# blasif/cocons

Hardware: AMD Instinct MI355X
Metric: -2loglik evals/sec (dense cov_rns + Cholesky/solve/log-det, fp64) at n=10000 (higher is better)
Workload: dtype f64

## Files before the change

cocons_amd/csrc/chol.hip:

```cpp
#include <hip/hip_runtime.h>
#include <limits.h>
#include <stdlib.h>
#include <string.h>
#include <algorithm>
#include <atomic>
#include <vector>
#include "kernels.h"

namespace cocons {

typedef double d4 __attribute__((ext_vector_type(4)));

#define MFMA64(a, b, c) __builtin_amdgcn_mfma_f64_16x16x4f64((a), (b), (c), 0, 0, 0)
#define MFMA64_NEGA(a, b, c) __builtin_amdgcn_mfma_f64_16x16x4f64((a), (b), (c), 0, 0, 1)

__device__ __forceinline__ void blk_mma(d4 &acc, const d4 &P, const d4 &Q)
{
    acc = MFMA64(Q[0], P[0], acc);
    acc = MFMA64(Q[1], P[1], acc);
    acc = MFMA64(Q[2], P[2], acc);
    acc = MFMA64(Q[3], P[3], acc);
}

__device__ __forceinline__ d4 lds_blk(const double *blk, int lane)
{
    d4 v;
    int o = (lane >> 4) * 16 + (lane & 15);
    v[0] = blk[o];
    v[1] = blk[o + 64];
    v[2] = blk[o + 128];
    v[3] = blk[o + 192];
    return v;
}

__device__ __forceinline__ void lds_blk_store(double *blk, int lane, const d4 &v)
{
    int o = (lane >> 4) * 16 + (lane & 15);
    blk[o] = v[0];
    blk[o + 64] = v[1];
    blk[o + 128] = v[2];
    blk[o + 192] = v[3];
}

__device__ __forceinline__ d4 glb_blk(const double *A, size_t lda, int row0, int col0, int lane)
{
    const double *p = A + (size_t)(row0 + (lane & 15)) + (size_t)(col0 + (lane >> 4)) * lda;
    d4 v;
    v[0] = p[0];
    v[1] = p[4 * lda];
    v[2] = p[8 * lda];
    v[3] = p[12 * lda];
    return v;
}

__device__ __forceinline__ void glb_blk_store(double *A, size_t lda, int row0, int col0, int lane, const d4 &v)
{
    double *p = A + (size_t)(row0 + (lane & 15)) + (size_t)(col0 + (lane >> 4)) * lda;
    p[0] = v[0];
    p[4 * lda] = v[1];
    p[8 * lda] = v[2];
    p[12 * lda] = v[3];
}

__device__ __forceinline__ void store_wt(double *p, double v)
{
    __hip_atomic_store((unsigned long long *)p, (unsigned long long)__double_as_longlong(v), __ATOMIC_RELAXED,
                       __HIP_MEMORY_SCOPE_AGENT);
}

__device__ __forceinline__ double load_wt(const double *p)
{
    return __longlong_as_double((long long)__hip_atomic_load((const unsigned long long *)p, __ATOMIC_RELAXED,
                                                             __HIP_MEMORY_SCOPE_AGENT));
}

__device__ __forceinline__ d4 glb_blk_wt(const double *A, size_t lda, int row0, int col0, int lane)
{
    const double *p = A + (size_t)(row0 + (lane & 15)) + (size_t)(col0 + (lane >> 4)) * lda;
    d4 v;
    v[0] = load_wt(p);
    v[1] = load_wt(p + 4 * lda);
    v[2] = load_wt(p + 8 * lda);
    v[3] = load_wt(p + 12 * lda);
    return v;
}

__device__ __forceinline__ void glb_blk_store_wt(double *A, size_t lda, int row0, int col0, int lane, const d4 &v)
{
    double *p = A + (size_t)(row0 + (lane & 15)) + (size_t)(col0 + (lane >> 4)) * lda;
    store_wt(p, v[0]);
    store_wt(p + 4 * lda, v[1]);
    store_wt(p + 8 * lda, v[2]);
    store_wt(p + 12 * lda, v[3]);
}

__device__ __forceinline__ double rdlane(double v, int lane)
{
    int lo = __builtin_amdgcn_readlane(__double2loint(v), lane);
    int hi = __builtin_amdgcn_readlane(__double2hiint(v), lane);
    return __hiloint2double(hi, lo);
}

__device__ __forceinline__ void rsqrt_pivot(double a, double &l, double &r)
{
    const double y0 = __builtin_amdgcn_rsq(a);
    const double s0 = a * y0;
    const double t = fma(-s0, y0, 1.0);
    const double y = fma(y0 * t, fma(t, 0.375, 0.5), y0);
    double s = a * y;
    s = fma(fma(-s, s, a), 0.5 * y, s);
    l = s;
    r = y;
}

__device__ __forceinline__ double sel_lower4(int c, int k, double v00, double v10, double v11, double v20,
                                             double v21, double v22, double v30, double v31, double v32, double v33)
{
    double r0 = v00;
    double r1 = (k == 0) ? v10 : v11;
    double r2 = (k == 0) ? v20 : ((k == 1) ? v21 : v22);
    double r3 = (k == 0) ? v30 : ((k == 1) ? v31 : ((k == 2) ? v32 : v33));
    double r = (c == 0) ? r0 : ((c == 1) ? r1 : ((c == 2) ? r2 : r3));
    return (k <= c) ? r : 0.0;
}

template <int S>
__device__ __forceinline__ void potrf16_step(d4 &D, double (&Q)[4], int lane, int &fail)
{
    const int m = lane & 15, k = lane >> 4;
    const double ds = D[S];
    double a00 = rdlane(ds, 4 * S + 0), a10 = rdlane(ds, 4 * S + 1), a20 = rdlane(ds, 4 * S + 2),
           a30 = rdlane(ds, 4 * S + 3);
    double a11 = rdlane(ds, 4 * S + 1 + 16), a21 = rdlane(ds, 4 * S + 2 + 16), a31 = rdlane(ds, 4 * S + 3 + 16);
    double a22 = rdlane(ds, 4 * S + 2 + 32), a32 = rdlane(ds, 4 * S + 3 + 32);
    double a33 = rdlane(ds, 4 * S + 3 + 48);
    double l00, r0;
    rsqrt_pivot(a00, l00, r0);
    double l10 = a10 * r0, l20 = a20 * r0, l30 = a30 * r0;
    double t11 = fma(-l10, l10, a11);
    double l11, r1;
    rsqrt_pivot(t11, l11, r1);
    double l21 = fma(-l20, l10, a21) * r1, l31 = fma(-l30, l10, a31) * r1;
    double t22 = fma(-l21, l21, fma(-l20, l20, a22));
    double l22, r2;
    rsqrt_pivot(t22, l22, r2);
    double l32 = fma(-l31, l21, fma(-l30, l20, a32)) * r2;
    double t33 = fma(-l32, l32, fma(-l31, l31, fma(-l30, l30, a33)));
    double l33, r3;
    rsqrt_pivot(t33, l33, r3);
    if (__builtin_amdgcn_ballot_w64(!(t33 > 0.0)) != 0ull && fail == 0)
        fail = 4 * S + (!(a00 > 0.0) ? 1 : (!(t11 > 0.0) ? 2 : (!(t22 > 0.0) ? 3 : 4)));
    double m00 = r0, m11 = r1, m22 = r2, m33 = r3;
    double m10 = -(l10 * m00) * r1;
    double m21 = -(l21 * m11) * r2;
    double m32 = -(l32 * m22) * r3;
    double m20 = -fma(l21, m10, l20 * m00) * r2;
    double m31 = -fma(l32, m21, l31 * m11) * r3;
    double m30 = -fma(l32, m20, fma(l31, m10, l30 * m00)) * r3;
    const int c = m & 3;
    const bool ingrp = (m >> 2) == S;
    double q = sel_lower4(c, k, m00, m10, m11, m20, m21, m22, m30, m31, m32, m33);
    q = ingrp ? q : 0.0;
    Q[S] = q;
    d4 z = {0.0, 0.0, 0.0, 0.0};
    d4 X = MFMA64(q, ds, z);
    (void)l11; (void)l22; (void)l33; (void)l00;
    double xs = (m < 4 * S + k) ? 0.0 : X[S];
    if (S < 3) {
        d4 U = MFMA64(xs, -xs, D);
#pragma unroll
        for (int r = S + 1; r < 4; ++r) D[r] = U[r];
    }
    D[S] = xs;
}

__device__ __forceinline__ int potrf16_regs(d4 &D, double (&Q)[4], int lane)
{
    int fail = 0;
    potrf16_step<0>(D, Q, lane, fail);
    potrf16_step<1>(D, Q, lane, fail);
    potrf16_step<2>(D, Q, lane, fail);
    potrf16_step<3>(D, Q, lane, fail);
    return fail;
}

__device__ __forceinline__ void trsm16(d4 &B, const d4 &L, const double (&Q)[4])
{
    const d4 z = {0.0, 0.0, 0.0, 0.0};
#pragma unroll
    for (int s = 0; s < 4; ++s) {
        d4 T = MFMA64(Q[s], B[s], z);
        B[s] = T[s];
        if (s < 3) {
            d4 U = MFMA64(L[s], -B[s], B);
#pragma unroll
            for (int r = s + 1; r < 4; ++r) B[r] = U[r];
        }
    }
}

__constant__ int c_tri_ib[36] = {0, 1, 1, 2, 2, 2, 3, 3, 3, 3, 4, 4, 4, 4, 4, 5, 5, 5, 5, 5, 5,
                                 6, 6, 6, 6, 6, 6, 6, 7, 7, 7, 7, 7, 7, 7, 7};

#ifndef POTRF_S_WAVES
#define POTRF_S_WAVES 7
#endif
#define MBOX_OFF(j) (256 * (9 * (j) - (j) * ((j) - 1) / 2))
__device__ __forceinline__ void mbox_store(double *mb, int lane, const d4 &v)
{
    store_wt(mb + lane, v[0]);
    store_wt(mb + lane + 64, v[1]);
    store_wt(mb + lane + 128, v[2]);
    store_wt(mb + lane + 192, v[3]);
}
template <bool WT, bool FROM_LDS = false>
__device__ __forceinline__ void potrf_tile_body(double *A, size_t lda, int c0, double *q_out, int *info, double *smem,
                                                double *qall, double *winv = nullptr, double *xi = nullptr, double *mbox = nullptr,
                                                unsigned *late = nullptr)
{
    const bool INV = winv != nullptr;
    double *S = smem;
    double *QS = smem + 36 * 256;
#define SB(ib, kb) (S + ((ib) * ((ib) + 1) / 2 + (kb)) * 256)
    int tid_ = threadIdx.x;
    asm volatile("" : "+v"(tid_));
    const int tid = tid_, lane = tid & 63, wave = __builtin_amdgcn_readfirstlane(tid >> 6);

    d4 D0 = {0.0, 0.0, 0.0, 0.0};
    double Q0[4] = {0.0, 0.0, 0.0, 0.0};
    if (FROM_LDS) {
        if (wave == 0) {
            D0 = lds_blk(S, lane);
            int f = potrf16_regs(D0, Q0, lane);
            if (f && lane == 0) atomicMin(info, c0 + f);
        }
    } else {
    if (wave == 0) {
#pragma unroll
        for (int r = 0; r < 4; ++r) {
            const int i = lane & 15, c = 4 * r + (lane >> 4);
            const double *sp = i < c ? A + (size_t)(c0 + c) + (size_t)(c0 + i) * lda : A + (size_t)(c0 + i) + (size_t)(c0 + c) * lda;
            D0[r] = WT ? load_wt(sp) : *sp;
        }
    }
    {
        const int i = tid & 15, k = (tid >> 4) & 15;
        const int half = __builtin_amdgcn_readfirstlane(tid >> 8);
        const double *src = A + (size_t)(c0 + i) + (size_t)(c0 + k) * lda;
        const double *srcd = (i < k) ? A + (size_t)(c0 + k) + (size_t)(c0 + i) * lda : src;
        double v[18];
#pragma unroll
        for (int t = 0; t < 18; ++t) {
            const int bb = 2 * t + half;
            const int ib = c_tri_ib[bb], kb = bb - ib * (ib + 1) / 2;
            const double *sp = (ib == kb ? srcd : src) + (size_t)(16 * ib) + (size_t)(16 * kb) * lda;
            v[t] = WT ? load_wt(sp) : *sp;
        }
        if (wave == 0) {
            int f = potrf16_regs(D0, Q0, lane);
            if (f && lane == 0) atomicMin(info, c0 + f);
        }
#pragma unroll
        for (int t = 0; t < 18; ++t) {
            const int bb = 2 * t + half;
            const int ib = c_tri_ib[bb], kb = bb - ib * (ib + 1) / 2;
            SB(ib, kb)[k * 16 + i] = v[t];
        }
    }
    }
    __syncthreads();
    if (wave == 0) {
        lds_blk_store(S, lane, D0);
        if (WT) glb_blk_store_wt(A, lda, c0, c0, lane, D0); else glb_blk_store(A, lda, c0, c0, lane, D0);
        if (mbox) mbox_store(mbox, lane, D0);
#pragma unroll
        for (int s = 0; s < 4; ++s) {
            QS[s * 64 + lane] = Q0[s];
            if (WT) store_wt(q_out + s * 64 + lane, Q0[s]); else q_out[s * 64 + lane] = Q0[s];
            if (qall) qall[s * 64 + lane] = Q0[s];
            if (mbox) store_wt(mbox + 8 * 256 + s * 64 + lane, Q0[s]);
        }
    }
    __syncthreads();

    for (int jb = 0; jb < 7; ++jb) {
        double *dblk = SB(jb, jb);
        double *qs = QS;
        if (jb + 1 + wave < 8) {
            const int ib = jb + 1 + wave;
            d4 L = lds_blk(dblk, lane);
            double Q[4];
#pragma unroll
            for (int s = 0; s < 4; ++s) Q[s] = qs[s * 64 + lane];
            double *blk = SB(ib, jb);
            d4 B = lds_blk(blk, lane);
            trsm16(B, L, Q);
            lds_blk_store(blk, lane, B);
            if (WT) glb_blk_store_wt(A, lda, c0 + 16 * ib, c0 + 16 * jb, lane, B);
            else glb_blk_store(A, lda, c0 + 16 * ib, c0 + 16 * jb, lane, B);
            if (mbox) mbox_store(mbox + MBOX_OFF(jb) + (ib - jb) * 256, lane, B);
        }
        __syncthreads();
        if (wave == 0) {
            const int nb = jb + 1;
            d4 P = lds_blk(SB(nb, jb), lane);
            double *blk = SB(nb, nb);
            d4 acc = lds_blk(blk, lane);
            d4 NP = -P;
            blk_mma(acc, NP, P);
            double Q[4];
            int f = potrf16_regs(acc, Q, lane);
            if (f && lane == 0) atomicMin(info, c0 + 16 * nb + f);
            if (late && jb == 0) asm volatile("s_waitcnt vmcnt(0)" ::: "memory");
            lds_blk_store(blk, lane, acc);
            if (WT) glb_blk_store_wt(A, lda, c0 + 16 * nb, c0 + 16 * nb, lane, acc);
            else glb_blk_store(A, lda, c0 + 16 * nb, c0 + 16 * nb, lane, acc);
            if (mbox) mbox_store(mbox + MBOX_OFF(nb), lane, acc);
// ... 958 lines not shown
        if (((row / (2 * TILE) / own_group) % own_world) != own_rank) return;
    }
    if (wait_word) {
        if (tid == 0) ok = wait_ge<false>(wait_word, 1u, abort_word, abort_code(ABORT_PANEL, (unsigned)(c0 / TILE))) ? 1 : 0;
        asm volatile("s_waitcnt vmcnt(0)" ::: "memory");
        __syncthreads();
        if (!ok) return;
        fetch_factor_tile<true>(A, lda, c0, qin, SL, QS, tid);
    } else
        fetch_factor_tile<false>(A, lda, c0, qin, SL, QS, tid);
    const int bx = blockIdx.x;
    const int rs = (bx < nb1 ? r0 + 64 * bx : e0 + 64 * (bx - nb1)) + 16 * wave;
    d4 B[8];
#pragma unroll
    for (int j = 0; j < 8; ++j) B[j] = glb_blk(A, lda, rs, c0 + 16 * j, lane);
    __syncthreads();
#pragma unroll
    for (int j = 0; j < 8; ++j) {
        d4 L = lds_blk(SL + (j * (j + 1) / 2 + j) * 256, lane);
        double Q[4];
#pragma unroll
        for (int s = 0; s < 4; ++s) Q[s] = QS[j * 256 + s * 64 + lane];
        trsm16(B[j], L, Q);
        d4 NX = -B[j];
#pragma unroll
        for (int jj = j + 1; jj < 8; ++jj) {
            d4 Lb = lds_blk(SL + (jj * (jj + 1) / 2 + j) * 256, lane);
            blk_mma(B[jj], NX, Lb);
        }
    }
#pragma unroll
    for (int j = 0; j < 8; ++j) glb_blk_store(A, lda, rs, c0 + 16 * j, lane, B[j]);
}


struct UpdArgs {
    double *C; size_t ldc;
    const double *P; size_t ldp;
    int K;
    int ti0, tj0, lower_only;
    int H, W;
    unsigned *sig; int sig_tile;
    unsigned *wait_word, *abort_word;
    int ptiles, world, rank;
    const int *pmap;
    int skip_lo, skip_hi;
    unsigned *queue; unsigned ntiles;
    int Hb, ext0;
    int c_wt;
    int skew, kblk;
};

template <int TM, int KC, int ROLE, int NW = 4>
__global__ void __launch_bounds__(64 * NW, 8)
update_kernel(UpdArgs a)
{
    constexpr int LDT = TM + 16;
    constexpr int WY = NW / 2;
    constexpr int NB = TM / 32;
    constexpr int NBY = TM / WY / 16;
    constexpr int TPC = 64 * NW / KC;
    constexpr int RPT = TM / TPC;
    __shared__ double sI[2][KC * LDT];
    __shared__ double sJ[2][KC * LDT];
    unsigned *share = (unsigned *)&sI[0][TM];
    const int tid = threadIdx.x;
    const int wave_s = __builtin_amdgcn_readfirstlane(tid >> 6);
    if (a.wait_word) {
        if (tid == 0) *share = wait_ge(a.wait_word, 1u, a.abort_word, abort_code(ABORT_INPANEL, (unsigned)a.tj0)) ? 1u : 0u;
        asm volatile("s_waitcnt vmcnt(0)" ::: "memory");
        __syncthreads();
        const unsigned ok = *share;
        __syncthreads();
        if (!ok) return;
    }

    else if (a.abort_word) {
        if (tid == 0) *share = __hip_atomic_load(a.abort_word, __ATOMIC_RELAXED, __HIP_MEMORY_SCOPE_AGENT);
        __syncthreads();
        const unsigned ab = *share;
        __syncthreads();
        if (ab) return;
    }

    const int nch = a.K / KC;
    typedef double d2 __attribute__((ext_vector_type(2)));

    unsigned L = blockIdx.x;
    for (;;) {
        int lane;
        asm volatile("v_mbcnt_lo_u32_b32 %0, -1, 0\n\tv_mbcnt_hi_u32_b32 %0, -1, %0" : "=v"(lane));
        const int wave = wave_s, t2 = 64 * wave + lane;
        const int wi = wave & 1, wj = wave >> 1;
        const int kc = t2 / TPC, rg = (t2 % TPC) * RPT;
        const int ro = (lane >> 4) * LDT + (lane & 15);
        int ti, tj;
        if (a.lower_only) {
            int lo = 0, hi = a.W - 1;
            while (lo < hi) {
                const int mid = (lo + hi + 1) >> 1;
                if (mid * a.H - mid * (mid - 1) / 2 <= (int)L) lo = mid; else hi = mid - 1;
            }
            const int j = lo;
            const int til = j + ((int)L - (j * a.H - j * (j - 1) / 2));
            tj = a.tj0 + j;
            ti = til < a.Hb ? a.tj0 + til : a.ext0 + (til - a.Hb);
        } else {
            const int til = blockIdx.x;
            ti = til < a.Hb ? a.ti0 + til : a.ext0 + (til - a.Hb);
            tj = a.tj0 + blockIdx.y;
        }
        if (a.world > 1 && ((ti * TM / (2 * TILE) / a.ptiles) % a.world) != a.rank) return;
        if (ti >= a.skip_lo && ti < a.skip_hi && tj >= a.skip_lo && tj < a.skip_hi) {
            if (!a.queue) return;
            if (t2 == 0) *share = gridDim.x + __hip_atomic_fetch_add(a.queue, 1u, __ATOMIC_RELAXED, __HIP_MEMORY_SCOPE_AGENT);
            __syncthreads();
            L = (unsigned)__builtin_amdgcn_readfirstlane((int)*share);
            __syncthreads();
            if (L >= a.ntiles) break;
            continue;
        }
        const int sig_Ti = (ti * TM) / TILE - a.sig_tile, sig_Tj = (tj * TM) / TILE - a.sig_tile;
        const bool sig_wg = a.sig != nullptr && sig_Ti >= 0 && sig_Ti <= 1 && sig_Tj >= 0 && sig_Tj <= sig_Ti;
        const bool wt_wg = sig_wg || a.c_wt;
        if (sig_wg) __builtin_amdgcn_s_setprio(3); else __builtin_amdgcn_s_setprio(0);

        int rowI_P = ti * TM, rowJ_P = tj * TM, rowI_C = ti * TM;
        if (a.pmap) { rowI_P = a.pmap[ti]; rowJ_P = a.pmap[tj]; }
        if (a.skew) {
            const bool ext = ti >= a.ext0;
            const int under = a.skew * TILE + (ti - a.ext0) * TM;
            rowI_P = ext ? under : ti * TM - TILE * a.kblk;
            rowJ_P = tj * TM - TILE * a.kblk;
            rowI_C = ext ? under : ti * TM - TILE * ((tj * TM) / TILE);
        }
        const double *gI = a.P + (size_t)(rowI_P + rg) + (size_t)kc * a.ldp;
        const double *gJ = a.P + (size_t)(rowJ_P + rg) + (size_t)kc * a.ldp;
        d2 stI[RPT / 2], stJ[RPT / 2];

        double *Cb = a.C + (size_t)(rowI_C + (TM / 2) * wi) + (size_t)(tj * TM + (TM / WY) * wj) * a.ldc;
        const unsigned ldcb = 8u * (unsigned)a.ldc;
        const unsigned cvo = 8u * (unsigned)(lane & 15) + (unsigned)(lane >> 4) * ldcb;
        d4 acc[NB][NBY];
#pragma unroll
        for (int x = 0; x < NB; ++x)
#pragma unroll
            for (int y = 0; y < NBY; ++y) acc[x][y] = (d4){0.0, 0.0, 0.0, 0.0};

#pragma unroll
        for (int v = 0; v < RPT / 2; ++v) {
            stI[v] = *(const d2 *)(gI + 2 * v);
            stJ[v] = *(const d2 *)(gJ + 2 * v);
        }
#pragma unroll
        for (int v = 0; v < RPT / 2; ++v) {
            *(d2 *)(&sI[0][kc * LDT + rg + 2 * v]) = stI[v];
            *(d2 *)(&sJ[0][kc * LDT + rg + 2 * v]) = stJ[v];
        }
        __syncthreads();

        for (int ch = 0; ch < nch; ++ch) {
            const int cur = ch & 1;
            if (ch + 1 < nch) {
                const double *pI = gI + (size_t)(ch + 1) * KC * a.ldp;
                const double *pJ = gJ + (size_t)(ch + 1) * KC * a.ldp;
#pragma unroll
                for (int v = 0; v < RPT / 2; ++v) {
                    stI[v] = *(const d2 *)(pI + 2 * v);
                    stJ[v] = *(const d2 *)(pJ + 2 * v);
                }
            }
            const double *bI = &sI[cur][ro + (TM / 2) * wi];
            const double *bJ = &sJ[cur][ro + (TM / WY) * wj];
#pragma unroll
            for (int s = 0; s < KC / 4; ++s) {
                double pi_[NB], pj_[NBY];
#pragma unroll
                for (int x = 0; x < NB; ++x) pi_[x] = bI[s * 4 * LDT + 16 * x];
#pragma unroll
                for (int y = 0; y < NBY; ++y) pj_[y] = bJ[s * 4 * LDT + 16 * y];
#pragma unroll
                for (int x = 0; x < NB; ++x)
#pragma unroll
                    for (int y = 0; y < NBY; ++y) acc[x][y] = MFMA64(pj_[y], pi_[x], acc[x][y]);
            }
            if (ch + 1 < nch) {
#pragma unroll
                for (int v = 0; v < RPT / 2; ++v) {
                    *(d2 *)(&sI[cur ^ 1][kc * LDT + rg + 2 * v]) = stI[v];
                    *(d2 *)(&sJ[cur ^ 1][kc * LDT + rg + 2 * v]) = stJ[v];
                }
            }
            __syncthreads();
        }
        unsigned Lnext = 0;
        if (a.queue && t2 == 0)
            Lnext = gridDim.x + __hip_atomic_fetch_add(a.queue, 1u, __ATOMIC_RELAXED, __HIP_MEMORY_SCOPE_AGENT);
        unsigned cve = cvo;
        asm volatile("" : "+v"(cve));
#pragma unroll
        for (int x = 0; x < NB; ++x)
#pragma unroll
            for (int y = 0; y < NBY; ++y) {
                d4 cv;
#pragma unroll
                for (int r = 0; r < 4; ++r) {
                    const double *cp = (const double *)((const char *)(Cb + 16 * x) + (cve + (unsigned)(16 * y + 4 * r) * ldcb));
                    cv[r] = a.c_wt ? load_wt(cp) : *cp;
                }
                cv -= acc[x][y];
                if (wt_wg) {
#pragma unroll
                    for (int r = 0; r < 4; ++r)
                        store_wt((double *)((char *)(Cb + 16 * x) + (cve + (unsigned)(16 * y + 4 * r) * ldcb)), cv[r]);
                } else {
#pragma unroll
                    for (int r = 0; r < 4; ++r)
                        *(double *)((char *)(Cb + 16 * x) + (cve + (unsigned)(16 * y + 4 * r) * ldcb)) = cv[r];
                }
            }
        if (wt_wg) {
            asm volatile("s_waitcnt vmcnt(0)" ::: "memory");
            __syncthreads();
            if (t2 == 0 && sig_wg) signal_add(a.sig + a.sig_tile + sig_Ti);
        }
        if (!a.queue) break;
        if (t2 == 0) *share = Lnext;
        __syncthreads();
        L = (unsigned)__builtin_amdgcn_readfirstlane((int)*share);
        if (L >= a.ntiles) break;
    }
}

struct DagStep {
    unsigned base;
    unsigned near;
    unsigned tpos, nT;
    int H, W;
    int tj0;
    int k0, K;
    int nstrip, two;
    int need;
    int nd_next;
    int split;
    unsigned p2, p3;
};

struct DagArgs {
    double *A; size_t lda;
    double *P;
    const double *Wt;
    const DagStep *steps; int nsteps;
    unsigned ntasks;
    unsigned *queue;
    unsigned *tdone;
    unsigned *pdone; int pstride;
    unsigned *pall;
    double *partbuf;
    unsigned *dcount;
    unsigned *sig;
    unsigned *out, *xr;
    unsigned *abort_word;
    const unsigned *alive;
    unsigned xcc_quota;
    unsigned *hw;
    unsigned long long *trace;
    const unsigned *ftab;
    unsigned xcd_g;
    unsigned *xcnt;
};

constexpr unsigned DAG_XCD_LAG = 64u;
__device__ __forceinline__ unsigned dag_position(unsigned c, unsigned cls, unsigned g)
{
    return ((c >> g) << (g + 3u)) | (cls << g) | (c & ((1u << g) - 1u));
}

__device__ __forceinline__ bool dag_wait(const DagArgs &a, unsigned *word, unsigned need, unsigned code, unsigned L)
{
    const unsigned long long t0 = __builtin_amdgcn_s_memrealtime();
    for (unsigned it = 0;; ++it) {
        const unsigned v = poll_word(word, it);
        if (v >= need) break;
        if (__hip_atomic_load(a.abort_word, __ATOMIC_RELAXED, __HIP_MEMORY_SCOPE_AGENT) != 0u) return false;
        if (it > (unsigned)(ENGINE_TIMEOUT_TICKS / 100ull) ||
            ((it & 1023u) == 1023u && __builtin_amdgcn_s_memrealtime() - t0 > WALL_BACKSTOP_TICKS)) {
            if (__hip_atomic_exchange(a.abort_word, code, __ATOMIC_RELAXED, __HIP_MEMORY_SCOPE_AGENT) == 0u) {
                unsigned *d = a.queue + 8;
                d[0] = L; d[1] = code; d[2] = (unsigned)(word - a.queue); d[3] = need; d[4] = v;
                d[5] = (unsigned)(__builtin_amdgcn_s_memrealtime() - t0);
                d[6] = it;
            }
            return false;
        }
        __builtin_amdgcn_s_sleep(16);
    }
    __builtin_amdgcn_fence(__ATOMIC_ACQUIRE, "wavefront");
    return true;
}

__global__ void __launch_bounds__(256, 8)
dag_kernel(DagArgs a)
{
    constexpr int TM = 64, KC = 8, LDT = TM + 16, TPC = 256 / KC, RPT = TM / TPC;
    static_assert(RPT == 2, "one 16-byte load per thread, side and chunk");
    typedef double d2 __attribute__((ext_vector_type(2)));
    __shared__ double sI[2][KC * LDT];
    __shared__ double sJ[2][KC * LDT];
    unsigned *share = (unsigned *)&sI[0][TM];
    const int tid = threadIdx.x;
    const int wave_s = __builtin_amdgcn_readfirstlane(tid >> 6);
    const DagStep *__restrict__ steps = a.steps;
    const unsigned ldab = 8u * (unsigned)a.lda;
    int known = 0;
    const unsigned myx = (hw_where() >> 28) & 7u;
    const bool loyal = ((blockIdx.x >> 3) & 1u) == 0u;
    if (tid == 0) {
        bool take = true;
        if (a.xcc_quota) {
            const unsigned c = __hip_atomic_load(a.alive + 16 + myx, __ATOMIC_RELAXED, __HIP_MEMORY_SCOPE_AGENT);
            if (c) {
                const unsigned less = 7u * (c - 1u);
                const unsigned quota = a.xcc_quota > less + 8u ? a.xcc_quota - less : 8u;
                take = __hip_atomic_fetch_add(a.queue + 16 + myx, 1u, __ATOMIC_RELAXED, __HIP_MEMORY_SCOPE_AGENT) < quota;
            }
        }
        unsigned first = 0xffffffffu;
        if (take) {
            if (a.xcd_g) first = dag_position(__hip_atomic_fetch_add(a.xcnt + 32u * myx, 1u, __ATOMIC_RELAXED, __HIP_MEMORY_SCOPE_AGENT), myx, a.xcd_g);
            else first = __hip_atomic_fetch_add(a.queue, 1u, __ATOMIC_RELAXED, __HIP_MEMORY_SCOPE_AGENT);
        }
        share[1] = first;
        share[2] = 0u;
    }
    __syncthreads();
    unsigned L = (unsigned)__builtin_amdgcn_readfirstlane((int)share[1]);
    __syncthreads();
    if (L >= a.ntasks) return;
    for (;;) {
        int lo = 0, hi = a.nsteps - 1;
        while (lo < hi) {
            const int mid = (lo + hi + 1) >> 1;
            if (steps[mid].base <= L) lo = mid; else hi = mid - 1;
        }
        const int s = lo;
        const DagStep st = steps[s];
        const unsigned q = L - st.base;
        if (a.trace && tid == 0) {
            a.trace[4 * (size_t)L] = __builtin_amdgcn_s_memrealtime();
            if (a.hw) a.hw[2 * (size_t)L] = hw_where();
        }
        const int t = st.tj0 >> 1;
        const unsigned per_u = 2u * (unsigned)st.nstrip, nA = per_u + (unsigned)st.nd_next, perBC = st.two ? per_u : 0u;
        int tkind = -1;
        unsigned tu = 0, qt_u = q;
        if (q >= st.tpos) {
            if (q < st.tpos + nA) { tu = q - st.tpos; tkind = tu < per_u ? 0 : 3; }
            else if (q < st.p2) qt_u = q - nA;
            else if (q < st.p2 + perBC) { tu = q - st.p2; tkind = 1; }
            else if (q < st.p3) qt_u = q - nA - perBC;
            else if (q < st.p3 + perBC) { tu = q - st.p3; tkind = 2; }
            else qt_u = q - nA - 2u * perBC;
        }
        const bool isT = tkind >= 0;
        const double *gIb, *gJb;
        unsigned ldib, ldjb, ldob = ldab;
        int K, i_wt = 0, store_only = 0, strip_task = 0;
        double *Cb;
        const double *pa = nullptr;
        unsigned *w0 = nullptr, *w1 = nullptr, *w2 = nullptr, *we = nullptr, *we2 = nullptr, *dn;
        unsigned n0 = 0, n1 = 0, n2 = 0, ne = 0, dval = 0;
        int sigT = -1;
        int prio = 0;
        if (!isT) {
            const int qt = (int)qt_u;
            int ti, tj;
            if (a.ftab && qt >= (int)st.near) {
                const unsigned e = a.ftab[a.ftab[s] + (unsigned)(qt - (int)st.near)];
                tj = st.tj0 + (int)(e & 0xffffu); ti = st.tj0 + (int)(e >> 16);
            } else {
                int jl = 0, jh = st.W - 1;
                while (jl < jh) {
                    const int mid = (jl + jh + 1) >> 1;
                    if (mid * st.H - mid * (mid - 1) / 2 <= qt) jl = mid; else jh = mid - 1;
                }
                tj = st.tj0 + jl; ti = tj + (qt - (jl * st.H - jl * (jl - 1) / 2));
            }
            const double *Ps = s == 0 ? a.A : a.P;
            gIb = Ps + (size_t)ti * TM + (size_t)st.k0 * a.lda;
            gJb = Ps + (size_t)tj * TM + (size_t)st.k0 * a.lda;
            ldib = ldab; ldjb = ldab; K = st.K;
            Cb = a.A + (size_t)ti * TM + (size_t)tj * TM * a.lda;
            if (s > known) {
                w0 = a.pall + s; n0 = (unsigned)st.H;
                w1 = a.pdone + (size_t)s * a.pstride + (ti - st.tj0); n1 = (unsigned)st.need;
                w2 = a.pdone + (size_t)s * a.pstride + (tj - st.tj0); n2 = (unsigned)st.need;
            }
            we = a.tdone + (ti * (ti + 1) / 2 + tj); ne = (unsigned)s;
            dn = we; dval = (unsigned)s + 1u;
            const int Ti = (ti >> 1) - t, Tj = (tj >> 1) - t;
            if (Ti >= 0 && Ti <= st.two && Tj >= 0 && Tj <= Ti) {
                sigT = t + Ti; prio = 3;
                if (st.split) {
                    const int ta = ti - st.tj0, tb = tj - st.tj0, dd = ta * (ta + 1) / 2 + tb;
                    gIb += (size_t)TILE * a.lda; gJb += (size_t)TILE * a.lda; K = TILE;
                    pa = a.partbuf + ((size_t)(s & 1) * 16 + dd) * (TM * TM);
                    we2 = a.dcount + (size_t)s * 16 + dd;
                }
            }
        } else {
            const int per = 2 * st.nstrip;
            const size_t c_t = (size_t)t * TILE, c_t1 = c_t + TILE;
            prio = 2;
            const int stage = tkind;
            int strip = 0, h = 0, row64 = 0;
            if (stage != 3) {
                strip = (int)(tu >> 1); h = (int)(tu & 1u);
                row64 = st.tj0 + (st.two ? 4 : 2) + strip;
                strip_task = 1;
            }
            dn = a.pdone + (size_t)(s + 1) * a.pstride + strip;
            if (stage == 3) {
                const int dd = (int)tu - per;
                const int ta = c_tri_ib[dd], tb = dd - ta * (ta + 1) / 2;
                const int tj0n = st.tj0 + 4;
                const size_t k0n = (size_t)(s + 1) * 2 * TILE;
                gIb = a.P + (size_t)(tj0n + ta) * TM + k0n * a.lda; ldib = ldab;
                gJb = a.P + (size_t)(tj0n + tb) * TM + k0n * a.lda; ldjb = ldab;
                K = TILE;
                Cb = a.partbuf + ((size_t)((s + 1) & 1) * 16 + dd) * (TM * TM); store_only = 1; ldob = 8u * TM;
                w0 = a.pdone + (size_t)(s + 1) * a.pstride + ta; n0 = 2u;
                w1 = a.pdone + (size_t)(s + 1) * a.pstride + tb; n1 = 2u;
                dn = a.dcount + (size_t)(s + 1) * 16 + dd;
            } else if (stage == 0) {
                gIb = a.A + (size_t)row64 * TM + c_t * a.lda; ldib = ldab; i_wt = 1;
                gJb = a.Wt + (size_t)t * TILE * TILE + TM * h; ldjb = 8u * TILE;
                K = TM * (h + 1);
                Cb = a.P + (size_t)row64 * TM + (c_t + TM * h) * a.lda; store_only = 1;
                w0 = a.out + t; n0 = 1u;
                w1 = a.tdone + (row64 * (row64 + 1) / 2 + 2 * t); n1 = (unsigned)s + 1u;
                w2 = w1 + 1; n2 = n1;
            } else if (stage == 1) {
                gIb = a.P + (size_t)row64 * TM + c_t * a.lda; ldib = ldab;
                gJb = a.P + (c_t1 + TM * h) + c_t * a.lda; ldjb = ldab;
                K = TILE;
                Cb = a.A + (size_t)row64 * TM + (c_t1 + TM * h) * a.lda;
                w0 = dn; n0 = 2u;
                w1 = a.xr + t; n1 = 1u;
                we = a.tdone + (row64 * (row64 + 1) / 2 + 2 * (t + 1) + h); ne = (unsigned)s + 1u;
            } else {
                gIb = a.A + (size_t)row64 * TM + c_t1 * a.lda; ldib = ldab; i_wt = 1;
                gJb = a.Wt + (size_t)(t + 1) * TILE * TILE + TM * h; ldjb = 8u * TILE;
                K = TM * (h + 1);
                Cb = a.P + (size_t)row64 * TM + (c_t1 + TM * h) * a.lda; store_only = 1;
                w0 = dn; n0 = 4u;
                w1 = a.out + t + 1; n1 = 1u;
            }
        }
        if (prio == 3) __builtin_amdgcn_s_setprio(3);
        else if (prio == 2) __builtin_amdgcn_s_setprio(2);
        else __builtin_amdgcn_s_setprio(0);

        if (w0) {
            if (tid == 0) {
                unsigned ok;
                if (!isT) {
                    if (__hip_atomic_load(w0, __ATOMIC_RELAXED, __HIP_MEMORY_SCOPE_AGENT) >= n0) ok = 2u;
                    else ok = (dag_wait(a, w1, n1, abort_code(0xb00u, (unsigned)s), L) &&
                               dag_wait(a, w2, n2, abort_code(0xc00u, (unsigned)s), L)) ? 1u : 0u;
                } else {
                    bool o = dag_wait(a, w0, n0, abort_code(0xa00u, (unsigned)s), L);
                    if (o && w1) o = dag_wait(a, w1, n1, abort_code(0xb00u, (unsigned)s), L);
                    if (o && w2) o = dag_wait(a, w2, n2, abort_code(0xc00u, (unsigned)s), L);
                    ok = o ? 1u : 0u;
                }
                *share = ok;
            }
            asm volatile("s_waitcnt vmcnt(0)" ::: "memory");
            __syncthreads();
            const unsigned ok = (unsigned)__builtin_amdgcn_readfirstlane((int)*share);
            __syncthreads();
            if (!ok) return;
            if (ok == 2u) known = s;
        }

        if (a.trace && tid == 0) a.trace[4 * (size_t)L + 1] = __builtin_amdgcn_s_memrealtime();
        int lane;
        asm volatile("v_mbcnt_lo_u32_b32 %0, -1, 0\n\tv_mbcnt_hi_u32_b32 %0, -1, %0" : "=v"(lane));
        const int wave = wave_s, t2 = 64 * wave + lane;
        const int wi = wave & 1, wj = wave >> 1;
        const int kc = t2 / TPC, rg = (t2 % TPC) * RPT;
        const int ro = (lane >> 4) * LDT + (lane & 15);
        const char *pI = (const char *)gIb + (8u * (unsigned)rg + (unsigned)kc * ldib);
        const char *pJ = (const char *)gJb + (8u * (unsigned)rg + (unsigned)kc * ldjb);
        const unsigned cIb = (unsigned)KC * ldib, cJb = (unsigned)KC * ldjb;
        const int nch = K / KC;
        d2 stI, stJ;
        d4 acc[2][2];
#pragma unroll
        for (int x = 0; x < 2; ++x)
#pragma unroll
            for (int y = 0; y < 2; ++y) acc[x][y] = (d4){0.0, 0.0, 0.0, 0.0};
        if (i_wt) { stI[0] = load_wt((const double *)pI); stI[1] = load_wt((const double *)pI + 1); }
        else stI = *(const d2 *)pI;
        stJ = *(const d2 *)pJ;
        *(d2 *)(&sI[0][kc * LDT + rg]) = stI;
        *(d2 *)(&sJ[0][kc * LDT + rg]) = stJ;
        __syncthreads();
        for (int ch = 0; ch < nch; ++ch) {
            const int cur = ch & 1;
            if (ch + 1 < nch) {
                const char *qI = pI + (unsigned)(ch + 1) * cIb;
                const char *qJ = pJ + (unsigned)(ch + 1) * cJb;
                if (i_wt) { stI[0] = load_wt((const double *)qI); stI[1] = load_wt((const double *)qI + 1); }
                else stI = *(const d2 *)qI;
                stJ = *(const d2 *)qJ;
            }
            const double *bI = &sI[cur][ro + (TM / 2) * wi];
            const double *bJ = &sJ[cur][ro + (TM / 2) * wj];
#pragma unroll
            for (int k4 = 0; k4 < KC / 4; ++k4) {
                const double p0 = bI[k4 * 4 * LDT], p1 = bI[k4 * 4 * LDT + 16];
                const double q0 = bJ[k4 * 4 * LDT], q1 = bJ[k4 * 4 * LDT + 16];
                acc[0][0] = MFMA64(q0, p0, acc[0][0]);
                acc[0][1] = MFMA64(q1, p0, acc[0][1]);
                acc[1][0] = MFMA64(q0, p1, acc[1][0]);
                acc[1][1] = MFMA64(q1, p1, acc[1][1]);
            }
            if (ch + 1 < nch) {
                *(d2 *)(&sI[cur ^ 1][kc * LDT + rg]) = stI;
                *(d2 *)(&sJ[cur ^ 1][kc * LDT + rg]) = stJ;
            }
            __syncthreads();
        }
        if (t2 == 0) {
            unsigned Ln, c = 0u, cy = 0u, cls = 0u, y = 0u;
            unsigned help = 0u;
            if (a.xcd_g) {
                help = loyal ? 0u : share[2];
                cls = help ? help - 1u : myx;
                y = help ? myx : ((myx + 1u + L % 7u) & 7u);
                c = __hip_atomic_fetch_add(a.xcnt + 32u * cls, 1u, __ATOMIC_RELAXED, __HIP_MEMORY_SCOPE_AGENT);
                cy = __hip_atomic_load(a.xcnt + 32u * y, __ATOMIC_RELAXED, __HIP_MEMORY_SCOPE_AGENT);
                Ln = 0u;
            } else
                Ln = __hip_atomic_fetch_add(a.queue, 1u, __ATOMIC_RELAXED, __HIP_MEMORY_SCOPE_AGENT);
            unsigned ok = 1u;
            if (we) ok = dag_wait(a, we, ne, abort_code(0xd00u, (unsigned)s), L) ? 1u : 0u;
            if (ok && we2) ok = wait_ge<false>(we2, 1u, a.abort_word, abort_code(0xe00u, (unsigned)s)) ? 1u : 0u;
            if (a.xcd_g) {
                Ln = dag_position(c, cls, a.xcd_g);
                if (!help) share[2] = (!loyal && c > cy + DAG_XCD_LAG && dag_position(cy, y, a.xcd_g) < a.ntasks) ? y + 1u : 0u;
                else {
                    share[2] = (c + DAG_XCD_LAG / 2u < cy && dag_position(c + 1u, cls, a.xcd_g) < a.ntasks) ? help : 0u;
                    if (Ln >= a.ntasks) {
                        cls = myx;
                        c = __hip_atomic_fetch_add(a.xcnt + 32u * cls, 1u, __ATOMIC_RELAXED, __HIP_MEMORY_SCOPE_AGENT);
                        Ln = dag_position(c, cls, a.xcd_g);
                    }
                }
                if (Ln >= a.ntasks && cls == myx) {
                    for (unsigned d = 1; d < 8u && Ln >= a.ntasks; ++d) {
                        const unsigned z = (myx + d) & 7u;
                        if (dag_position(__hip_atomic_load(a.xcnt + 32u * z, __ATOMIC_RELAXED, __HIP_MEMORY_SCOPE_AGENT), z, a.xcd_g) < a.ntasks)
                            Ln = dag_position(__hip_atomic_fetch_add(a.xcnt + 32u * z, 1u, __ATOMIC_RELAXED, __HIP_MEMORY_SCOPE_AGENT), z, a.xcd_g);
                    }
                }
            }
            share[0] = ok; share[1] = Ln;
            if (a.trace) a.trace[4 * (size_t)L + 2] = __builtin_amdgcn_s_memrealtime();
        }
        asm volatile("s_waitcnt vmcnt(0)" ::: "memory");
        __syncthreads();
        const unsigned okE = share[0];
        const unsigned Lnext = share[1];
        if (!okE) return;
        double *Cw = (double *)((char *)(Cb + (TM / 2) * wi) + (size_t)((TM / 2) * wj) * ldob);
        unsigned cve = 8u * (unsigned)(lane & 15) + (unsigned)(lane >> 4) * ldob;
        asm volatile("" : "+v"(cve));
#pragma unroll
        for (int x = 0; x < 2; ++x)
#pragma unroll
            for (int y = 0; y < 2; ++y) {
                d4 cv;
                if (store_only) cv = acc[x][y];
                else {
#pragma unroll
                    for (int r = 0; r < 4; ++r)
                        cv[r] = load_wt((const double *)((const char *)(Cw + 16 * x) + (cve + (unsigned)(16 * y + 4 * r) * ldob)));
                    if (pa) {
                        const double *Pw = pa + (TM / 2) * wi + (TM / 2) * wj * TM;
                        int ln;
                        asm volatile("v_mbcnt_lo_u32_b32 %0, -1, 0\n\tv_mbcnt_hi_u32_b32 %0, -1, %0" : "=v"(ln));
                        const unsigned cvp = 8u * (unsigned)(ln & 15) + (unsigned)(ln >> 4) * (8u * TM);
                        d4 pv;
#pragma unroll
                        for (int r = 0; r < 4; ++r)
                            pv[r] = load_wt((const double *)((const char *)(Pw + 16 * x) + (cvp + (unsigned)(16 * y + 4 * r) * (8u * TM))));
                        cv -= pv + acc[x][y];
                    } else cv -= acc[x][y];
                }
#pragma unroll
                for (int r = 0; r < 4; ++r)
                    store_wt((double *)((char *)(Cw + 16 * x) + (cve + (unsigned)(16 * y + 4 * r) * ldob)), cv[r]);
            }
        asm volatile("s_waitcnt vmcnt(0)" ::: "memory");
        __syncthreads();
        if (t2 == 0) {
            if (sigT >= 0) signal_add(a.sig + sigT);
            if (dval) __hip_atomic_fetch_max(dn, dval, __ATOMIC_RELAXED, __HIP_MEMORY_SCOPE_AGENT);
            else if (__hip_atomic_fetch_add(dn, 1u, __ATOMIC_RELAXED, __HIP_MEMORY_SCOPE_AGENT) + 1u == (st.two ? 6u : 2u) && strip_task)
                __hip_atomic_fetch_add(a.pall + s + 1, 1u, __ATOMIC_RELAXED, __HIP_MEMORY_SCOPE_AGENT);
            if (a.trace) {
                a.trace[4 * (size_t)L + 3] = __builtin_amdgcn_s_memrealtime();
                if (a.hw) a.hw[2 * (size_t)L + 1] = hw_where();
            }
        }
        L = (unsigned)__builtin_amdgcn_readfirstlane((int)Lnext);
        if (L >= a.ntasks) break;
    }
}

__device__ __forceinline__ double block_sum(double v, double *red)
{
#pragma unroll
    for (int o = 32; o > 0; o >>= 1) v += __shfl_down(v, o, 64);
    int lane = threadIdx.x & 63, wave = threadIdx.x >> 6;
    if (lane == 0) red[wave] = v;
    __syncthreads();
    double t = 0.0;
    if (threadIdx.x == 0)
        for (int w = 0; w < (int)(blockDim.x >> 6); ++w) t += red[w];
    __syncthreads();
    return t;
}

__global__ void __launch_bounds__(1024)
finalize_kernel(const double *A, size_t lda, int c0, int c1, int n, int row0, int nr, double *out, int skew, int npad,
                const double *A2, int a2_cols)
{
    __shared__ double red[16];
    const int b = blockIdx.x;
    const int hi = c1 < n ? c1 : n;
    double s = 0.0;
    constexpr int U = 4;
    const int step = (int)blockDim.x;
    if (b == nr * nr) {
        for (int c = c0 + (int)threadIdx.x; c < hi; c += U * step) {
            double v[U];
#pragma unroll
            for (int q = 0; q < U; ++q) v[q] = (c + q * step < hi) ? A[band_index(c + q * step, c + q * step, lda, skew, npad)] : 1.0;
#pragma unroll
            for (int q = 0; q < U; ++q) s += log(v[q]);
        }
    } else {
        const int ra = row0 + b / nr, rb = row0 + b % nr;
        for (int c = c0 + (int)threadIdx.x; c < hi; c += U * step) {
            double va[U], vb[U];
#pragma unroll
            for (int q = 0; q < U; ++q) {
                const bool in = c + q * step < hi;
                const int cc = c + q * step;
                int below0 = 2 * TILE * (cc / (2 * TILE) + 1);
                if (npad > 0 && below0 > npad) below0 = npad;
                const bool in2 = A2 && cc >= 2 * TILE && cc < a2_cols;
                const double *Sa = (in2 && ra >= below0) ? A2 : A;
                const double *Sb = (in2 && rb >= below0) ? A2 : A;
                va[q] = in ? Sa[band_index(ra, cc, lda, skew, npad)] : 0.0;
                vb[q] = in ? Sb[band_index(rb, cc, lda, skew, npad)] : 0.0;
            }
#pragma unroll
            for (int q = 0; q < U; ++q) s += va[q] * vb[q];
        }
    }
    s = block_sum(s, red);
    if (threadIdx.x == 0) out[b == nr * nr ? 0 : 1 + b] = s;
}

__global__ void __launch_bounds__(256)
row_reduce_kernel(const double *A, size_t lda, int n, int rowy, int row0, int m,
                  double *scratch, int cchunk, int skew, int npad, const double *A2, int a2_cols)
{
    const int i = blockIdx.x * blockDim.x + threadIdx.x;
    const int cb = blockIdx.y * cchunk;
    const int ce = (cb + cchunk < n) ? cb + cchunk : n;
    if (i >= m) return;
    if (A2 && cb >= 2 * TILE && cb < a2_cols) A = A2;
    double s = 0.0, q = 0.0;
    for (int c = cb; c < ce; ++c) {
        double v = A[band_index(row0 + i, c, lda, skew, npad)];
        double y = A[band_index(rowy, c, lda, skew, npad)];
        s = fma(v, y, s);
        q = fma(v, v, q);
    }
    scratch[((size_t)blockIdx.y * 2 + 0) * m + i] = s;
    scratch[((size_t)blockIdx.y * 2 + 1) * m + i] = q;
}

__global__ void __launch_bounds__(256)
row_reduce_final_kernel(const double *scratch, int m, int nchunks, double *stoch, double *quad)
{
    const int i = blockIdx.x * blockDim.x + threadIdx.x;
    if (i >= m) return;
    double s = 0.0, q = 0.0;
    for (int c = 0; c < nchunks; ++c) {
        s += scratch[((size_t)c * 2 + 0) * m + i];
        q += scratch[((size_t)c * 2 + 1) * m + i];
    }
    stoch[i] = s;
    quad[i] = q;
}

__global__ void __launch_bounds__(256)
trmm_lower_kernel(const double *A, size_t lda, int n, const double *E, int lde, int nsim,
                  const double *trend, double *Y, int ldy)
{
    __shared__ double red[4][8][64];
    const int lane = threadIdx.x & 63, wave = threadIdx.x >> 6;
    const int rb = gridDim.x - 1 - blockIdx.x;
    const int i = rb * 64 + lane;
    const int kend = (rb + 1) * 64 < n ? (rb + 1) * 64 : n;
    for (int s0 = 0; s0 < nsim; s0 += 8) {
        double acc[8] = {0, 0, 0, 0, 0, 0, 0, 0};
        for (int k = wave; k < kend; k += 4) {
            double l = (i < n && k <= i) ? A[(size_t)i + (size_t)k * lda] : 0.0;
#pragma unroll
            for (int s = 0; s < 8; ++s)
                if (s0 + s < nsim) acc[s] = fma(l, E[(size_t)k + (size_t)(s0 + s) * lde], acc[s]);
        }
#pragma unroll
        for (int s = 0; s < 8; ++s) red[wave][s][lane] = acc[s];
        __syncthreads();
        if (wave == 0 && i < n) {
#pragma unroll
            for (int s = 0; s < 8; ++s)
                if (s0 + s < nsim)
                    Y[(size_t)i + (size_t)(s0 + s) * ldy] =
                        ((red[0][s][lane] + red[1][s][lane]) + (red[2][s][lane] + red[3][s][lane])) + trend[i];
        }
        __syncthreads();
    }
}

void launch_trmm_lower(const double *A, size_t lda, int n, const double *E, int lde, int nsim,
                       const double *trend, double *Y, int ldy, hipStream_t s)
{
    if (n <= 0 || nsim <= 0) return;
    hipLaunchKernelGGL(trmm_lower_kernel, dim3((n + 63) / 64), dim3(256), 0, s, A, lda, n, E, lde, nsim, trend, Y, ldy);
}

constexpr int BT_COLS = 64;
constexpr size_t BT_LDS_BYTES = (size_t)TILE * BT_COLS * sizeof(double);

__device__ __forceinline__ int bt_lds_index(int k, int j)
{
    return (((k >> 4) * (BT_COLS / 16) + (j >> 4)) << 8) + ((k & 15) << 4) + ((j ^ k) & 15);
}

__global__ void __launch_bounds__(256)
band_trmm_kernel(const double *A, size_t lda, int skew, int npad, const int *hi, int n, const double *E, int lde,
                 int nsim, const double *trend, double *Y, int ldy)
{
    extern __shared__ double Es[];
    const int I = blockIdx.x, s0 = blockIdx.y * BT_COLS;
    const int lane = threadIdx.x & 63, wave = threadIdx.x >> 6;
    int c0 = 0;
    if (hi) {
        int lo = 0, up = I;
        while (lo < up) {
            const int mid = (lo + up) >> 1;
            if (hi[mid] > I) up = mid; else lo = mid + 1;
        }
        c0 = lo;
    }
    d4 acc[2][4];
#pragma unroll
    for (int rb = 0; rb < 2; ++rb)
#pragma unroll
        for (int jb = 0; jb < 4; ++jb) acc[rb][jb] = d4{0.0, 0.0, 0.0, 0.0};
    const int row0 = I * TILE + 32 * wave;
    for (int c = c0; c <= I; ++c) {
        __syncthreads();
        for (int e = threadIdx.x; e < TILE * BT_COLS; e += 256) {
            const int k = e & (TILE - 1), j = e >> 7;
            const int gk = c * TILE + k, gj = s0 + j;
            Es[bt_lds_index(k, j)] = (gk < n && gj < nsim) ? E[(size_t)gk + (size_t)gj * lde] : 0.0;
        }
        __syncthreads();
        const double *Ac = skew ? A - (ptrdiff_t)TILE * c : A;
        const bool diag = c == I;
#pragma unroll
        for (int kb = 0; kb < TILE / 16; ++kb) {
            if (diag && kb > 2 * wave + 1) break;
            d4 P[2];
#pragma unroll
            for (int rb = 0; rb < 2; ++rb) {
                const int lb = 2 * wave + rb;
                if (diag && kb > lb) { P[rb] = d4{0.0, 0.0, 0.0, 0.0}; continue; }
                P[rb] = glb_blk(Ac, lda, row0 + 16 * rb, c * TILE + 16 * kb, lane);
                if (diag && kb == lb) {
#pragma unroll
                    for (int r = 0; r < 4; ++r)
                        if (4 * r + (lane >> 4) > (lane & 15)) P[rb][r] = 0.0;
                }
            }
#pragma unroll
            for (int jb = 0; jb < 4; ++jb) {
                const double *blk = Es + ((kb * (BT_COLS / 16) + jb) << 8);
                d4 Q;
#pragma unroll
                for (int r = 0; r < 4; ++r) {
                    const int k = (lane >> 4) + 4 * r, j = lane & 15;
                    Q[r] = blk[(k << 4) + ((j ^ k) & 15)];
                }
                blk_mma(acc[0][jb], P[0], Q);
                blk_mma(acc[1][jb], P[1], Q);
            }
        }
    }
#pragma unroll
    for (int rb = 0; rb < 2; ++rb) {
        const int i = row0 + 16 * rb + (lane & 15);
        if (i >= n) continue;
        const double t = trend[i];
#pragma unroll
        for (int jb = 0; jb < 4; ++jb)
#pragma unroll
            for (int r = 0; r < 4; ++r) {
                const int j = s0 + 16 * jb + 4 * r + (lane >> 4);
                if (j < nsim) Y[(size_t)i + (size_t)j * ldy] = acc[rb][jb][r] + t;
            }
    }
}

static void set_dynamic_lds_once(const void *kernel, size_t bytes, std::atomic<unsigned long long> &done_mask);
void launch_band_trmm(const double *A, size_t lda, int skew, int npad, const int *d_hi, int nt, int n, const double *E,
                      int lde, int nsim, const double *trend, double *Y, int ldy, hipStream_t s)
// ... 602 lines not shown
```

Baseline: 119.2.

## Stream DAG GEMM tiles via global_load_lds into a 4-deep LDS ring

Replaces the register-staged double-buffered load/store of the I and J panels in the DAG tile kernel with direct global-to-LDS loads (global_load_lds) into a four-slot ring with KC=4. Loads run three chunks ahead, tracked by vmcnt waits. Waves 0-1 fetch I and waves 2-3 fetch J, with an XOR swizzle on the LDS layout. This removes the VGPR round-trip and the LDS store instructions, and makes global latency hiding deeper. In exchange there are more barriers per K element, since each chunk now holds 4 instead of 8. Correctness depends on hand-managed waitcnt ordering, and the loop assumes nch is a multiple of RING.

New measurement: 124.2, median of 6. +4.2%, better.

```diff
diff --git a/cocons_amd/csrc/chol.hip b/cocons_amd/csrc/chol.hip
--- a/cocons_amd/csrc/chol.hip
+++ b/cocons_amd/csrc/chol.hip
@@ -13,6 +13,7 @@
 
 #define MFMA64(a, b, c) __builtin_amdgcn_mfma_f64_16x16x4f64((a), (b), (c), 0, 0, 0)
 #define MFMA64_NEGA(a, b, c) __builtin_amdgcn_mfma_f64_16x16x4f64((a), (b), (c), 0, 0, 1)
+#define LDS_T __attribute__((address_space(3)))
 
 __device__ __forceinline__ void blk_mma(d4 &acc, const d4 &P, const d4 &Q)
 {
@@ -1577,12 +1578,9 @@
 __global__ void __launch_bounds__(256, 8)
 dag_kernel(DagArgs a)
 {
-    constexpr int TM = 64, KC = 8, LDT = TM + 16, TPC = 256 / KC, RPT = TM / TPC;
-    static_assert(RPT == 2, "one 16-byte load per thread, side and chunk");
-    typedef double d2 __attribute__((ext_vector_type(2)));
-    __shared__ double sI[2][KC * LDT];
-    __shared__ double sJ[2][KC * LDT];
-    unsigned *share = (unsigned *)&sI[0][TM];
+    constexpr int TM = 64, KC = 4, RING = 4, STG = 2 * KC * TM;
+    __shared__ double smem[RING * STG + 2];
+    unsigned *share = (unsigned *)&smem[RING * STG];
     const int tid = threadIdx.x;
     const int wave_s = __builtin_amdgcn_readfirstlane(tid >> 6);
     const DagStep *__restrict__ steps = a.steps;
@@ -1764,50 +1762,52 @@
         asm volatile("v_mbcnt_lo_u32_b32 %0, -1, 0\n\tv_mbcnt_hi_u32_b32 %0, -1, %0" : "=v"(lane));
         const int wave = wave_s, t2 = 64 * wave + lane;
         const int wi = wave & 1, wj = wave >> 1;
-        const int kc = t2 / TPC, rg = (t2 % TPC) * RPT;
-        const int ro = (lane >> 4) * LDT + (lane & 15);
-        const char *pI = (const char *)gIb + (8u * (unsigned)rg + (unsigned)kc * ldib);
-        const char *pJ = (const char *)gJb + (8u * (unsigned)rg + (unsigned)kc * ldjb);
-        const unsigned cIb = (unsigned)KC * ldib, cJb = (unsigned)KC * ldjb;
+        const bool opJ = wave >= 2;
+        const char *gsrc = opJ ? (const char *)gJb : (const char *)gIb;
+        const unsigned ldg = opJ ? ldjb : ldib, cstep = (unsigned)KC * ldg;
+        const bool wt = i_wt && !opJ;
+        const int sc = (lane >> 5) & 1;
+        const char *src = gsrc + ((unsigned)(2 * (wave & 1) + sc) * ldg + 8u * (unsigned)((2 * (lane & 31)) ^ (16 * sc)));
+        LDS_T double *ldst = (LDS_T double *)(smem + 128 * wave);
         const int nch = K / KC;
-        d2 stI, stJ;
+#define DAG_STAGE(slot)                                                                                                     \
+        do {                                                                                                                \
+            if (wt) __builtin_amdgcn_global_load_lds((const void *)src, (LDS_T void *)(ldst + STG * (slot)), 16, 0, 16);   \
+            else __builtin_amdgcn_global_load_lds((const void *)src, (LDS_T void *)(ldst + STG * (slot)), 16, 0, 0);       \
+            src += cstep;                                                                                                   \
+        } while (0)
+        const int kq = lane >> 4, kodd = kq & 1, rl = (lane & 15) + TM * kq;
+        const int aI0 = rl + (TM / 2) * wi + 16 * kodd, aI1 = rl + (TM / 2) * wi + 16 * (kodd ^ 1);
+        const int aJ0 = KC * TM + rl + (TM / 2) * wj + 16 * kodd, aJ1 = KC * TM + rl + (TM / 2) * wj + 16 * (kodd ^ 1);
         d4 acc[2][2];
 #pragma unroll
         for (int x = 0; x < 2; ++x)
 #pragma unroll
             for (int y = 0; y < 2; ++y) acc[x][y] = (d4){0.0, 0.0, 0.0, 0.0};
-        if (i_wt) { stI[0] = load_wt((const double *)pI); stI[1] = load_wt((const double *)pI + 1); }
-        else stI = *(const d2 *)pI;
-        stJ = *(const d2 *)pJ;
-        *(d2 *)(&sI[0][kc * LDT + rg]) = stI;
-        *(d2 *)(&sJ[0][kc * LDT + rg]) = stJ;
-        __syncthreads();
-        for (int ch = 0; ch < nch; ++ch) {
-            const int cur = ch & 1;
-            if (ch + 1 < nch) {
-                const char *qI = pI + (unsigned)(ch + 1) * cIb;
-                const char *qJ = pJ + (unsigned)(ch + 1) * cJb;
-                if (i_wt) { stI[0] = load_wt((const double *)qI); stI[1] = load_wt((const double *)qI + 1); }
-                else stI = *(const d2 *)qI;
-                stJ = *(const d2 *)qJ;
-            }
-            const double *bI = &sI[cur][ro + (TM / 2) * wi];
-            const double *bJ = &sJ[cur][ro + (TM / 2) * wj];
-#pragma unroll
-            for (int k4 = 0; k4 < KC / 4; ++k4) {
-                const double p0 = bI[k4 * 4 * LDT], p1 = bI[k4 * 4 * LDT + 16];
-                const double q0 = bJ[k4 * 4 * LDT], q1 = bJ[k4 * 4 * LDT + 16];
+        DAG_STAGE(0);
+        DAG_STAGE(1);
+        DAG_STAGE(2);
+        for (int c0 = 0; c0 < nch; c0 += RING) {
+#pragma unroll
+            for (int r = 0; r < RING; ++r) {
+                const int ch = c0 + r;
+                if (ch + 2 < nch) asm volatile("s_waitcnt vmcnt(2)" ::: "memory");
+                else if (ch + 1 < nch) asm volatile("s_waitcnt vmcnt(1)" ::: "memory");
+                else asm volatile("s_waitcnt vmcnt(0)" ::: "memory");
+                asm volatile("s_waitcnt lgkmcnt(0)" ::: "memory");
+                __builtin_amdgcn_s_barrier();
+                asm volatile("" ::: "memory");
+                if (ch + RING - 1 < nch) DAG_STAGE((r + RING - 1) % RING);
+                const double *bs = smem + STG * r;
+                const double p0 = bs[aI0], p1 = bs[aI1];
+                const double q0 = bs[aJ0], q1 = bs[aJ1];
                 acc[0][0] = MFMA64(q0, p0, acc[0][0]);
                 acc[0][1] = MFMA64(q1, p0, acc[0][1]);
                 acc[1][0] = MFMA64(q0, p1, acc[1][0]);
                 acc[1][1] = MFMA64(q1, p1, acc[1][1]);
             }
-            if (ch + 1 < nch) {
-                *(d2 *)(&sI[cur ^ 1][kc * LDT + rg]) = stI;
-                *(d2 *)(&sJ[cur ^ 1][kc * LDT + rg]) = stJ;
-            }
-            __syncthreads();
-        }
+        }
+#undef DAG_STAGE
         if (t2 == 0) {
             unsigned Ln, c = 0u, cy = 0u, cls = 0u, y = 0u;
             unsigned help = 0u;
```
